# parsakzr/medvae-disentangled-multimodal

Measured on AMD Instinct MI355X. Metric: training images/sec (whole node) + ELBO parity, multimodal CVAE 64×64 bs=256, higher is better.
Workload: dtype fp32 (3xBF16 MFMA, fp32 accumulate); 1 GPU; ConditionalVAE 64x64x3 train step (fwd+loss+bwd+clip+adamw); model=ConditionalVAE, params=927333315, global_batch=256, per_gpu_batch=256, resolution=64, parallelism=dp1, rccl_world_size=1, step_launch=eager

## Files before the change

include/medvae_hip.h:

```cpp
#ifndef MEDVAE_HIP_H
#define MEDVAE_HIP_H

#include <stddef.h>

#ifdef __cplusplus
extern "C" {
#endif

#define MVAE_OK 0
#define MVAE_EINVAL (-1)
#define MVAE_EWORKSPACE (-2)

const char* mvae_last_error(void);
int mvae_abi_version(void);

int mvae_set_math_mode(int mode);
int mvae_get_math_mode(void);
int mvae_set_dropout_salt(const void* salt_dev);

#define MVAE_CONV_WSPLIT 16
#define MVAE_CONV_XSPLIT 32
#define MVAE_CONV_DYSPLIT 64
#define MVAE_CONV_BF16 128
#define MVAE_CONV_PLANAR 256
// ... 40 lines not shown
int mvae_conv2d_wgrad_upsample_nhwc(const float* dy, const float* x, float* dw, float* dbias, float beta, int nb,
                                    int h, int w_, int cin, int cout, float* workspace, size_t workspace_bytes,
                                    void* stream);
size_t mvae_conv2d_wgrad_upsample_workspace_bytes(int nb, int h, int w_, int cin, int cout);

int mvae_winograd_weight_transform(const float* w, void* u, int cin, int cout, int dgrad, int tile, void* stream);
int mvae_winograd_input_transform(const float* x, void* v, int nb, int h, int w, int c, int x_split, int tile,
                                  void* stream);
int mvae_winograd_input_transform_gn(const float* x, const float* scale, const float* shift, int silu, void* v, int nb,
                                     int h, int w, int c, int tile, void* stream);
int mvae_winograd_gemm(const void* v, const void* u, float* m, long long tiles, int k_in, int n_out, int tile,
                       void* stream);
int mvae_winograd_output_transform(const float* m, const float* bias, const float* residual, float* y, double* gn_part,
                                   int nb, int h, int w, int n, int tile, void* stream);
int mvae_winograd_output_gnbwd(const float* m, float* dx, const float* x, const float* mean, const float* rstd,
                               const float* gamma, const float* beta, int groups, int silu, double* part, int nb, int h,
                               int w, int n, int tile, void* stream);
int mvae_winograd_dy_transform(const float* dy, void* d, int nb, int h, int w, int k, int dy_split, int tile,
                               void* stream);
int mvae_winograd_dy_transforms(const float* dy, void* v, void* d, int nb, int h, int w, int k, int dy_split, int tile,
                                void* stream);
int mvae_winograd_wgrad_gemm(const void* d, const void* v, float* m, long long tiles, int cout, int cin, int tile,
                             float* workspace, size_t workspace_bytes, void* stream);
int mvae_winograd_wgrad_output(const float* m, float* dw, float beta, int cout, int cin, int tile, void* stream);
int mvae_winograd_upsample_weights(const float* w, float* kc, int cin, int cout, void* stream);
int mvae_winograd_upsample_fold(const float* dkc, float* dw, float beta, int cin, int cout, void* stream);
int mvae_winograd_output_transform_upsample(const float* m, const float* bias, float* y, int nb, int h, int w, int cout,
                                            int tile, void* stream);
int mvae_winograd_dy_transforms_upsample(const float* dy, void* v, void* d, int nb, int h, int w, int cout, int tile,
                                         void* stream);

int mvae_split_bf16(const float* x, void* y, long long n, void* stream);
int mvae_pack_bf16(const float* x, void* y, long long n, void* stream);
int mvae_pack_bf16_colsum(const float* x, void* y, long long rows, int n, float* out, float beta, void* workspace,
                          size_t workspace_bytes, void* stream);
int mvae_split_planar(const float* x, void* y, long long n, void* stream);
int mvae_split_planar_colsum(const float* x, void* y, long long rows, int n, float* out, float beta, void* workspace,
                             size_t workspace_bytes, void* stream);

int mvae_conv_weight_transpose(const float* w, float* wt, int cout, int kh, int kw, int cin, int split, void* stream);
typedef struct {
  const float* w;
  float* wt;
  int cout, rs, cin, split;
  int block0, pad0;
} mvae_wt_desc;
int mvae_conv_weight_transpose_batched(const mvae_wt_desc* table, int n, int total_blocks, void* stream);
// ... 183 lines not shown
```

medvae_disentangled_multimodal_amd/_lib.py:

```python
from __future__ import annotations

import ctypes
import os
from ctypes import c_double, c_float, c_int, c_longlong, c_size_t, c_uint64, c_void_p

_HERE = os.path.dirname(os.path.abspath(__file__))
LIB_PATH = os.environ.get("MVAE_HIP_LIB", os.path.join(_HERE, "libmvae_hip.so"))

P = c_void_p
I = c_int
L = c_longlong
F = c_float
D = c_double
Z = c_size_t

SIGNATURES = {
    "mvae_last_error": (ctypes.c_char_p, []),
    "mvae_abi_version": (I, []),
    "mvae_set_math_mode": (I, [I]),
    "mvae_get_math_mode": (I, []),
    "mvae_set_dropout_salt": (I, [P]),
    "mvae_conv2d_nhwc": (I, [P, P, P, P, P, I, I, I, I, I, I, I, I, I, I, I, I, I, P]),
    "mvae_conv2d_direct32_nhwc": (I, [P, P, P, P, P, I, I, I, I, P]),
    "mvae_conv2d_ws_nhwc": (I, [P, P, P, P, P, I, I, I, I, I, I, I, I, I, I, I, I, I, P, Z, P]),
    "mvae_conv2d_split_workspace_bytes": (Z, [I, I, I, I, I, I, I]),
    "mvae_conv2d_gnstats_nhwc": (I, [P, P, P, P, P, I, I, I, I, I, I, I, I, I, I, I, I, I, P, P]),
    "mvae_conv2d_dgrad_gnbwd_nhwc": (I, [P, P, P, I, I, I, I, I, I, I, I, I, I, I, I, P, P, P, P, P, I, I, P, P]),
    "mvae_conv2d_wgrad_nhwc": (I, [P, P, P, P, F, I, I, I, I, I, I, I, I, I, I, I, I, I, P, Z, P]),
    "mvae_winograd_weight_transform": (I, [P, P, I, I, I, I, P]),
    "mvae_winograd_input_transform": (I, [P, P, I, I, I, I, I, I, P]),
    "mvae_winograd_input_transform_gn": (I, [P, P, P, I, P, I, I, I, I, I, P]),
    "mvae_group_norm_stats_nhwc": (I, [P, P, P, P, P, P, P, P, I, I, I, I, F, P, Z, P]),
    "mvae_group_norm_apply_nhwc": (I, [P, P, P, P, I, I, I, I, I, P]),
    "mvae_winograd_gemm": (I, [P, P, P, L, I, I, I, P]),
    "mvae_winograd_output_transform": (I, [P, P, P, P, P, I, I, I, I, I, P]),
    "mvae_winograd_output_gnbwd": (I, [P, P, P, P, P, P, P, I, I, P, I, I, I, I, I, P]),
    "mvae_winograd_dy_transform": (I, [P, P, I, I, I, I, I, I, P]),
    "mvae_winograd_dy_transforms": (I, [P, P, P, I, I, I, I, I, I, P]),
    "mvae_winograd_wgrad_gemm": (I, [P, P, P, L, I, I, I, P, Z, P]),
    "mvae_winograd_wgrad_output": (I, [P, P, F, I, I, I, P]),
    "mvae_winograd_upsample_weights": (I, [P, P, I, I, P]),
    "mvae_winograd_upsample_fold": (I, [P, P, F, I, I, P]),
    "mvae_winograd_output_transform_upsample": (I, [P, P, P, I, I, I, I, I, P]),
    "mvae_winograd_dy_transforms_upsample": (I, [P, P, P, I, I, I, I, I, P]),
    "mvae_conv2d_wgrad_workspace_bytes": (Z, [I, I, I, I, I, I, I]),
    "mvae_conv2d_wgrad_small_cout_nhwc": (I, [P, P, P, P, F, I, I, I, I, I, I, P, Z, P]),
    "mvae_conv2d_wgrad_small_cout_workspace_bytes": (Z, [I, I]),
    "mvae_conv2d_wgrad_direct_nhwc": (I, [P, P, P, P, F, I, I, I, I, I, I, P, Z, P]),
    "mvae_conv2d_wgrad_direct_workspace_bytes": (Z, [I, I, I, I, I]),
    "mvae_conv_weight_transpose": (I, [P, P, I, I, I, I, I, P]),
    "mvae_conv_weight_transpose_batched": (I, [P, I, I, P]),
    "mvae_conv_weight_upsample_dgrad": (I, [P, P, I, I, I, P]),
    "mvae_conv2d_dgrad_stride2_nhwc": (I, [P, P, P, I, I, I, I, I, I, I, I, I, I, I, I, P, Z, P]),
    "mvae_split_bf16": (I, [P, P, L, P]),
    "mvae_pack_bf16": (I, [P, P, L, P]),
    "mvae_pack_bf16_colsum": (I, [P, P, L, I, P, F, P, Z, P]),
    "mvae_split_planar": (I, [P, P, L, P]),
    "mvae_split_planar_colsum": (I, [P, P, L, I, P, F, P, Z, P]),
    "mvae_conv2d_upsample_nhwc": (I, [P, P, P, P, P, I, I, I, I, I, I, P]),
    "mvae_conv_weight_upsample_fwd": (I, [P, P, I, I, I, P]),
    "mvae_conv2d_wgrad_upsample_nhwc": (I, [P, P, P, P, F, I, I, I, I, I, P, Z, P]),
    "mvae_conv2d_wgrad_upsample_workspace_bytes": (Z, [I, I, I, I, I]),
    "mvae_bias_grad": (I, [P, L, I, L, P, F, P, Z, P]),
# ... 141 lines not shown
```

medvae_disentangled_multimodal_amd/csrc/gemm_core.h:

```cpp
#pragma once
#include "common.h"
#include <algorithm>
#include <stdlib.h>
#include <type_traits>

namespace mvae {

enum { A_ROWK = 0, A_COLM = 1, A_CONV_FWD = 2, A_CONV_UPS = 3, A_CONV_DGRAD = 4, A_CONV_SUBPIX = 5, A_COLM_PIX = 6,
       A_CONV_FWD_SPLIT = 7, A_CONV_DGRAD_SPLIT = 8, A_COLM_SPLIT = 9, A_ROWK_SPLIT = 10 };
enum { B_ROWK = 0, B_COLN = 1, B_WGRAD_FWD = 2, B_WGRAD_UPS = 3, B_WGRAD_SUBPIX = 4, B_ROWK_SPLIT = 5,
       B_WGRAD_FWD_SPLIT = 6, B_WGRAD_P2 = 7, B_WGRAD_P2_SPLIT = 8, B_COLN_SPLIT = 9 };
enum { MODE_FWD = 0, MODE_UPS = 1, MODE_DGRAD = 2, MODE_SUBPIX = 3 };

constexpr int BK = 32;
template <int MF> using acc_of = typename std::conditional<MF == 32, f32x16, f32x4>::type;
template <int MF> constexpr int ks_of() { return BK / (MF == 32 ? 16 : 32); }
template <int MF> constexpr int nr_of() { return MF == 32 ? 16 : 4; }
__device__ __forceinline__ int row_swz(int r) { return ((r >> 2) ^ (r >> 3) ^ (r >> 4)) & 1; }
__device__ __forceinline__ int col_swz(int kr) { return ((kr >> 3) & 1) << 4; }
__device__ __forceinline__ int row_off(int r, int kc) { return r * 40 + (((kc >> 1) ^ row_swz(r)) << 3) + ((kc & 1) << 2); }
constexpr int MVAE_CONV_WSPLIT = 16;
constexpr int MVAE_CONV_XSPLIT = 32;
constexpr int MVAE_CONV_DYSPLIT = 64;
constexpr int MVAE_CONV_BF16 = 128;
constexpr int MVAE_CONV_PLANAR = 256;
constexpr int MVAE_CONV_DGRAD_DIRECT = 512;

struct Magic {
  unsigned m;
  int sh;
};
inline Magic make_magic(int d) {
  int l = 0;
  while ((1LL << l) < d) ++l;
  return Magic{(unsigned)(((1ULL << (31 + l)) / (unsigned long long)d) + 1ULL), 31 + l};
}
__device__ __forceinline__ int mdiv(int n, Magic mg) {
  return (int)(((unsigned long long)(unsigned)n * mg.m) >> mg.sh);
}

struct GemmArgs {
  int M, N, K;
  int batch, splits, k_split;
  const float* A; long long lda, sA;
  const float* B; long long ldb, sB;
  float* C; long long ldc, sC;
// ... 1587 lines not shown
    }
  }
}

template <int BM, int BN, int WGM, int WGN, int AK, int VA, int BKIND, int VB, int PREC>
__global__ void __launch_bounds__(64 * WGM * WGN) gemm3x_persist_kernel(GemmArgs a) {
  constexpr int NT = 64 * WGM * WGN;
  constexpr int MF = (MVAE_COL_MF16 && mf_of(AK) == 32) ? 16 : mf_of(AK);
  static_assert(MF == 16 && (PREC == 0 || PREC == 3), "persistent GEMM: 16x16x32 tiles, 3xBF16 or exact fp32");
  constexpr int KS = ks_of<MF>(), NR = nr_of<MF>();
  using acc_t = acc_of<MF>;
  using LA = Loader<AK, BM, VA, NT, true, PREC>;
  using LB = Loader<BKIND, BN, VB, NT, false, PREC>;
  using IA = Img<BM, LA::COL>;
  using IB = Img<BN, LB::COL>;
  constexpr int BUF = IA::SIZE + IB::SIZE;
  constexpr int TM = BM / WGM / MF, TN = BN / WGN / MF;
  static_assert(TM % 2 == 0, "persistent GEMM: the 16-B epilogue stages half of the wave's rows at a time");
  __shared__ __attribute__((aligned(16))) __bf16 lds[2 * BUF];

  const int tid = threadIdx.x, lane = tid & 63, wid = tid >> 6;
  const int wm = wid / WGN, wn = wid - wm * WGN;
  const int arow = wm * (BM / WGM), brow = wn * (BN / WGN);
  const int ntile = a.tiles_m * a.tiles_n, total = ntile * a.batch, grid = (int)gridDim.x;
  int lin = blockIdx.x;
  if (grid >= 16) {
    const int xcd = lin & 7, q = grid >> 3, r = grid & 7;
    lin = (xcd < r ? xcd * (q + 1) : r * (q + 1) + (xcd - r) * q) + (lin >> 3);
  }
  auto locate = [&](int l, int& m0, int& n0, int& bidx) {
    bidx = l / ntile;
    const int tile = l - bidx * ntile;
    int tm, tn;
    if (a.xcd_groups > 1 && a.tiles_n > 1) {
      const int gw = (a.tiles_n + a.xcd_groups - 1) / a.xcd_groups;
      const int ng = (a.tiles_n + gw - 1) / gw;
      const int g = min(tile / (a.tiles_m * gw), ng - 1);
      const int rem = tile - g * a.tiles_m * gw;
      const int width = g == ng - 1 ? a.tiles_n - g * gw : gw;
      tm = rem / width;
      tn = g * gw + (rem - tm * width);
    } else {
      tm = tile / a.tiles_n;
      tn = tile - tm * a.tiles_n;
    }
    m0 = tm * BM;
    n0 = tn * BN;
  };
  const int nt = (a.K + BK - 1) / BK;

  LA la;
  LB lb;
  auto prefetch = [&](int l) {
    int m0, n0, bidx;
    locate(l, m0, n0, bidx);
    la.init(a, a.A + bidx * a.sA, m0, 0, tid, bidx);
    lb.init(a, a.B + bidx * a.sB, n0, 0, tid, bidx);
    la.load(a);
    lb.load(a);
  };
  acc_t acc[TM][TN];
  auto compute = [&](const __bf16* Ai) {
    const __bf16* Bi = Ai + IA::SIZE;
#pragma unroll
    for (int ks = 0; ks < KS; ++ks) {
      bf16x8 bh[TN], bl[TN];
#pragma unroll
      for (int j = 0; j < TN; ++j) {
        bh[j] = read_frag<BN, LB::COL, MF>(Bi, brow + j * MF, ks, lane);
        bl[j] = read_frag<BN, LB::COL, MF>(Bi + IB::PLANE, brow + j * MF, ks, lane);
      }
#pragma unroll
      for (int i = 0; i < TM; ++i) {
        const bf16x8 ah = read_frag<BM, LA::COL, MF>(Ai, arow + i * MF, ks, lane);
        const bf16x8 al = read_frag<BM, LA::COL, MF>(Ai + IA::PLANE, arow + i * MF, ks, lane);
#pragma unroll
        for (int j = 0; j < TN; ++j) mma<PREC>(acc[i][j], ah, al, bh[j], bl[j]);
      }
    }
  };

  prefetch(lin);
  for (int l = lin;;) {
    int m0, n0, bidx;
    locate(l, m0, n0, bidx);
    const int lnext = l + grid;
    const bool more = lnext < total;
#pragma unroll
    for (int i = 0; i < TM; ++i)
#pragma unroll
      for (int j = 0; j < TN; ++j)
#pragma unroll
        for (int r = 0; r < NR; ++r) acc[i][j][r] = 0.f;
    la.store(lds);
    lb.store(lds + IA::SIZE);
    if (nt > 1) {
      la.advance();
      lb.advance();
      la.load(a);
      lb.load(a);
    }
    __syncthreads();
    int t = 0;
    constexpr int STEPS = KS * TM;
    constexpr int NSL = LA::NS + LB::NS;
#ifndef MVAE_NO_PRIO
    if (NT >= 512 && wid >= (NT / 64) / 2) __builtin_amdgcn_s_setprio(1);
#endif
// ... 41 lines not shown
            bh[j] = read_frag<BN, LB::COL, MF>(Bi, brow + j * MF, 1, lane);
            bl[j] = read_frag<BN, LB::COL, MF>(Bi + IB::PLANE, brow + j * MF, 1, lane);
          }
        }
        stage(st);
        __builtin_amdgcn_sched_barrier(0);
      }
      __syncthreads();
    }
#ifndef MVAE_NO_PRIO
    __builtin_amdgcn_s_setprio(0);
#endif
    if (t + 1 < nt) {
      __bf16* nb = lds + ((t & 1) ^ 1) * BUF;
      la.store(nb);
      lb.store(nb + IA::SIZE);
      compute(lds + (t & 1) * BUF);
      __syncthreads();
      ++t;
    }
    compute(lds + (t & 1) * BUF);
    if (more) prefetch(lnext);

    {
      constexpr int WR = BM / WGM, WC = BN / WGN, HR = WR / 2, PE = WC + 4;
      static_assert((NT / 64) * HR * PE * 4 <= 4 * BUF, "epilogue staging exceeds the LDS");
      constexpr int C4 = WC / 4, RPI = 64 / C4;
      float* stg = (float*)lds + wid * HR * PE;
      const __amdgpu_buffer_rsrc_t cr = make_rsrc(a.C + bidx * a.sC, a.c_bytes);
      const int c4 = lane % C4, rsub = lane / C4;
      const int col = n0 + brow + c4 * 4;
      __syncthreads();
#pragma unroll
      for (int pass = 0; pass < 2; ++pass) {
#pragma unroll
        for (int i = 0; i < TM / 2; ++i)
#pragma unroll
          for (int j = 0; j < TN; ++j)
#pragma unroll
            for (int r = 0; r < NR; ++r)
              stg[(i * 16 + acc_row<MF>(r, lane)) * PE + j * 16 + (lane & 15)] = acc[pass * (TM / 2) + i][j][r];
        __syncthreads();
#pragma unroll
        for (int k = 0; k < HR / RPI; ++k) {
          const int lr = k * RPI + rsub;
          const float4 s4 = *(const float4*)(stg + lr * PE + c4 * 4);
// ... 292 lines not shown
```

medvae_disentangled_multimodal_amd/csrc/winograd.hip:

```cpp
#include "gemm_core.h"

namespace mvae {

__device__ __forceinline__ float4 f4add(float4 a, float4 b) { return float4{a.x + b.x, a.y + b.y, a.z + b.z, a.w + b.w}; }

template <int MT>
__host__ __device__ constexpr float wino_bt(int i, int j) {
  if constexpr (MT == 2) {
    constexpr float m[4][4] = {{1, 0, -1, 0}, {0, 1, 1, 0}, {0, -1, 1, 0}, {0, 1, 0, -1}};
    return m[i][j];
  } else {
    constexpr float m[6][6] = {{4, 0, -5, 0, 1, 0},  {0, -4, -4, 1, 1, 0}, {0, 4, -4, -1, 1, 0},
                               {0, -2, -1, 2, 1, 0}, {0, 2, -1, -2, 1, 0}, {0, 4, 0, -5, 0, 1}};
    return m[i][j];
  }
}
template <int MT>
__host__ __device__ constexpr float wino_g(int i, int j) {
  if constexpr (MT == 2) {
    constexpr float m[4][3] = {{1, 0, 0}, {0.5f, 0.5f, 0.5f}, {0.5f, -0.5f, 0.5f}, {0, 0, 1}};
    return m[i][j];
  } else {
    constexpr float m[6][3] = {{0.25f, 0, 0},
                               {-1.f / 6, -1.f / 6, -1.f / 6},
// ... 577 lines not shown
#pragma unroll
  for (int i = 0; i < AL; ++i)
#pragma unroll
    for (int j = 0; j < AL; ++j) mv[i][j] = bload4(mr, (unsigned)(t * K4 + k4) * 16u + (unsigned)(i * AL + j) * mplane);
  constexpr auto at = [](int i, int k) { return wino_at<MT>(i, k); };
  float4 r[MT][AL];
#pragma unroll
  for (int j = 0; j < AL; ++j) wlin<MT, AL>(&r[0][j], AL, &mv[0][j], AL, at);
#pragma unroll
  for (int a = 0; a < MT; ++a) {
    float4 o[MT];
    wlin<MT, AL>(o, 1, &r[a][0], 1, at);
    const int row = ti * MT + a;
#pragma unroll
    for (int e = 0; e < MT; ++e) {
      const int col = tj * MT + e;
      const unsigned off =
          ((unsigned)((b * 2 * p.H + 2 * row + (pq >> 1)) * 2 * p.W + 2 * col + (pq & 1)) * (unsigned)N + c4 * 4) * 4u;
      bstore4(yr, (row < p.H && col < p.W) ? off : OOB, f4add(o[e], bv));
    }
  }
}

template <int MT>
__global__ void __launch_bounds__(256) wino_wout_kernel(const float* __restrict__ m, float* __restrict__ dw, float beta,
                                                        int cout, int cin) {
  constexpr int AL = MT + 2;
  const int C4 = cin >> 2;
  const long long idx = (long long)blockIdx.x * blockDim.x + threadIdx.x;
  if (idx >= (long long)cout * C4) return;
  const long long mn = (long long)cout * cin;
  float4 mv[AL][AL];
#pragma unroll
  for (int i = 0; i < AL; ++i)
#pragma unroll
    for (int j = 0; j < AL; ++j) mv[i][j] = *(const float4*)(m + (i * AL + j) * mn + idx * 4);
  constexpr auto gt = [](int r, int i) { return wino_g<MT>(i, r); };
  float4 r[3][AL], o[3][3];
#pragma unroll
  for (int j = 0; j < AL; ++j) wlin<3, AL>(&r[0][j], AL, &mv[0][j], AL, gt);
#pragma unroll
  for (int i = 0; i < 3; ++i) wlin<3, AL>(&o[i][0], 1, &r[i][0], 1, gt);
  const int k = (int)(idx / C4), c4 = (int)(idx - (long long)k * C4);
#pragma unroll
  for (int i = 0; i < 3; ++i)
#pragma unroll
    for (int j = 0; j < 3; ++j) {
      float4* q = (float4*)(dw + (((long long)k * 3 + i) * 3 + j) * cin + c4 * 4);
      float4 val = o[i][j];
      if (beta != 0.f) {
        const float4 old = *q;
        val = float4{fmaf(beta, old.x, val.x), fmaf(beta, old.y, val.y), fmaf(beta, old.z, val.z),
                     fmaf(beta, old.w, val.w)};
      }
      *q = val;
    }
}

static long long wino_tiles(int nb, int h, int w, int mt) {
  return (long long)nb * ((h + mt - 1) / mt) * ((w + mt - 1) / mt);
}

static bool wino_geom_ok(int mt, int nb, int h, int w, int cin, int cout) {
// ... 90 lines not shown
    if (tile == 2) hipLaunchKernelGGL(wino_out_any_kernel<2>, g, dim3(256), 0, st, p);
    else hipLaunchKernelGGL(wino_out_any_kernel<4>, g, dim3(256), 0, st, p);
    return launch_status();
  }
  const int wseg = std::min(p.W, 32);
  if (tile == 2) {
    if (wseg == 8) wino_out_go<2, 8>(p, gnb, st);
    else if (wseg == 16) wino_out_go<2, 16>(p, gnb, st);
    else wino_out_go<2, 32>(p, gnb, st);
  } else {
    if (wseg == 8) wino_out_go<4, 8>(p, gnb, st);
    else if (wseg == 16) wino_out_go<4, 16>(p, gnb, st);
    else wino_out_go<4, 32>(p, gnb, st);
  }
  return launch_status();
}

template <int CFG, int AK, int BKIND>
static bool persist_cfg(GemmArgs& a, hipStream_t st) {
  constexpr int BM = 256, BN = CFG == T256x256 ? 256 : 128;
  constexpr int WGM = CFG == T256x128 ? 4 : 2, WGN = CFG == T256x256 ? 4 : 2;
  a.tiles_m = cdiv(a.M, BM);
  a.tiles_n = cdiv(a.N, BN);
  const long long total = (long long)a.tiles_m * a.tiles_n * a.batch, slots = 256LL * resident_of(CFG);
  if (total <= slots || total > (1LL << 30)) return false;
  if (a.xcd_groups <= 0) a.xcd_groups = xcd_groups_env();
  const dim3 grid((unsigned)slots), block(64 * WGM * WGN);
  if (math_mode() == MATH_FP32) {
    if constexpr (CFG == T256x256) return false;
    else hipLaunchKernelGGL((gemm3x_persist_kernel<BM, BN, WGM, WGN, AK, 4, BKIND, 4, 0>), grid, block, 0, st, a);
  } else {
    hipLaunchKernelGGL((gemm3x_persist_kernel<BM, BN, WGM, WGN, AK, 4, BKIND, 4, 3>), grid, block, 0, st, a);
  }
  return true;
}
template <int AK, int BKIND>
static bool launch_persist(GemmArgs& a, hipStream_t st, int cfg) {
  static_assert(AK == A_ROWK_SPLIT && BKIND == B_ROWK_SPLIT, "persistent GEMM: pre-split ROW x ROW operands");
#ifdef MVAE_W4
  return false;
#else
  if (getenv("MVAE_NO_PERSISTENT_GEMM") != nullptr || math_mode() == MATH_BF16 || a.splits != 1 || a.bias || a.res ||
      a.beta != 0.f || a.out_remap || a.gn_part || a.gnb_part || a.bias_ws || (a.N & 3) || (a.ldc & 3) || (a.sC & 3) ||
      !al16(a.C) || vec_epi_disabled())
    return false;
  if (cfg == T256x256) return persist_cfg<T256x256, AK, BKIND>(a, st);
  if (cfg == T256x128) return persist_cfg<T256x128, AK, BKIND>(a, st);
  return false;
#endif
}

}

using namespace mvae;

extern "C" {

int mvae_winograd_weight_transform(const float* w, void* u, int cin, int cout, int dgrad, int tile, void* stream) {
  if (!w || !u || cin <= 0 || cout <= 0 || cin % 4 || cout % 4 || !al16(w) || !al16(u) || (tile != 2 && tile != 4)) {
    set_error("winograd_weight_transform: cin, cout multiples of 4, 16-B aligned w / u, tile 2 or 4");
    return MVAE_EINVAL;
  }
  hipStream_t st = (hipStream_t)stream;
  const int sf = wino_sf();
  if (tile == 2) WINO_GO(wt_go, 2, w, u, cin, cout, dgrad, st);
  else WINO_GO(wt_go, 4, w, u, cin, cout, dgrad, st);
  return launch_status();
}

int mvae_winograd_input_transform(const float* x, void* v, int nb, int h, int w, int c, int x_split, int tile,
                                  void* stream) {
  if (!x || !v || !wino_geom_ok(tile, nb, h, w, c, c) || !al16(x) || !al16(v)) {
// ... 116 lines not shown
  hipStream_t st = (hipStream_t)stream;
  const int sf = wino_sf();
  if (tile == 2) WINO_GO(dy_go, 2, dy, nullptr, d, nb, h, w, k, dy_split, false, st);
  else WINO_GO(dy_go, 4, dy, nullptr, d, nb, h, w, k, dy_split, false, st);
  return launch_status();
}

int mvae_winograd_dy_transforms(const float* dy, void* v, void* d, int nb, int h, int w, int k, int dy_split, int tile,
                                void* stream) {
  if (!dy || !v || !d || !wino_geom_ok(tile, nb, h, w, k, k) || !al16(dy) || !al16(v) || !al16(d)) {
    set_error("winograd_dy_transforms: tile 2 or 4, k %% 4 == 0, 16-B aligned");
    return MVAE_EINVAL;
  }
  if (!wino_split_in_ok(dy_split)) return MVAE_EINVAL;
  hipStream_t st = (hipStream_t)stream;
  const int sf = wino_sf();
  if (tile == 2) WINO_GO(dy_go, 2, dy, v, d, nb, h, w, k, dy_split, true, st);
  else WINO_GO(dy_go, 4, dy, v, d, nb, h, w, k, dy_split, true, st);
  return launch_status();
}

int mvae_winograd_wgrad_gemm(const void* d, const void* v, float* m, long long tiles, int cout, int cin, int tile,
                             float* workspace, size_t workspace_bytes, void* stream) {
  if (!d || !v || !m || tiles <= 0 || cout <= 0 || cin <= 0 || cout % 4 || cin % 4 || !al16(d) || !al16(v) || !al16(m) ||
      tiles * std::max(cout, cin) * 4 > MAX_DESC_BYTES || tiles > (1LL << 30) || (tile != 2 && tile != 4)) {
    set_error("winograd_wgrad_gemm: cout, cin multiples of 4, 16-B aligned, one position < 4 GiB, tile 2 or 4");
    return MVAE_EINVAL;
  }
  const bool pk = wino_sf() == 2;
  if (pk && (cout % 8 || cin % 8)) {
    set_error("winograd_wgrad_gemm: the bf16 (packed) operands need cout, cin %% 8 == 0");
    return MVAE_EINVAL;
  }
  const unsigned eb = pk ? 2u : 4u;
  GemmArgs a{};
  a.M = cout; a.N = cin; a.K = (int)tiles; a.batch = (tile + 2) * (tile + 2);
  a.A = (const float*)d; a.lda = cout; a.sA = tiles * cout;
  a.B = (const float*)v; a.ldb = cin; a.sB = tiles * cin;
  a.C = m; a.ldc = cin; a.sC = (long long)cout * cin;
  a.alpha = 1.f; a.beta = 0.f;
  a.a_bytes = (unsigned)(tiles * cout * eb); a.b_bytes = (unsigned)(tiles * cin * eb);
  a.c_bytes = (unsigned)((long long)cout * cin * 4);
  const int cfg = choose_tile(a, true, workspace != nullptr);
  plan_splits(a, cfg, workspace, workspace_bytes);
  if (pk) wgrad_dma(B_COLN, a, (hipStream_t)stream, cfg, 4);
  else launch_big<A_COLM_SPLIT, 4, B_COLN_SPLIT, 4>(a, (hipStream_t)stream, cfg);
  return gemm_finish(a, (hipStream_t)stream);
}

int mvae_winograd_upsample_weights(const float* w, float* kc, int cin, int cout, void* stream) {
  if (!w || !kc || cin <= 0 || cout <= 0 || cin % 4 || !al16(w) || !al16(kc)) {
    set_error("winograd_upsample_weights: cin %% 4 == 0, 16-B aligned");
    return MVAE_EINVAL;
  }
  hipLaunchKernelGGL(wino_ups_weights_kernel, dim3(egrid256(4LL * cout * (cin / 4))), dim3(256), 0, (hipStream_t)stream,
                     w, kc, cout, cin);
  return launch_status();
}

int mvae_winograd_upsample_fold(const float* dkc, float* dw, float beta, int cin, int cout, void* stream) {
  if (!dkc || !dw || cin <= 0 || cout <= 0 || cin % 4 || !al16(dkc) || !al16(dw)) {
    set_error("winograd_upsample_fold: cin %% 4 == 0, 16-B aligned");
    return MVAE_EINVAL;
  }
  hipLaunchKernelGGL(wino_ups_fold_kernel, dim3(egrid256((long long)cout * (cin / 4))), dim3(256), 0,
                     (hipStream_t)stream, dkc, dw, beta, cout, cin);
  return launch_status();
}

int mvae_winograd_output_transform_upsample(const float* m, const float* bias, float* y, int nb, int h, int w, int cout,
// ... 6 lines not shown
  WinoOut p{};
  p.m = m; p.bias = bias; p.y = y;
  p.groups = 1; p.nb = nb; p.H = h; p.W = w; p.N = cout;
  const dim3 g(egrid256(wino_tiles(nb, h, w, tile) * cout));
  if (tile == 2) hipLaunchKernelGGL(wino_out_ups_kernel<2>, g, dim3(256), 0, (hipStream_t)stream, p);
  else hipLaunchKernelGGL(wino_out_ups_kernel<4>, g, dim3(256), 0, (hipStream_t)stream, p);
  return launch_status();
}

int mvae_winograd_dy_transforms_upsample(const float* dy, void* v, void* d, int nb, int h, int w, int cout, int tile,
                                         void* stream) {
  if (!dy || !d || cout % 4 || !wino_geom_ok(tile, nb, h, w, 4 * cout, 4 * cout) || !al16(dy) || !al16(d) ||
      (v && !al16(v))) {
    set_error("winograd_dy_transforms_upsample: tile 2 or 4, cout %% 4 == 0, 16-B aligned, operands < 4 GiB");
    return MVAE_EINVAL;
  }
  hipStream_t st = (hipStream_t)stream;
  const int sf = wino_sf(), k = 4 * cout;
  if (tile == 2) WINO_GO(dy_go, 2, dy, v, d, nb, h, w, k, 0, v != nullptr, st, true);
  else WINO_GO(dy_go, 4, dy, v, d, nb, h, w, k, 0, v != nullptr, st, true);
  return launch_status();
}

int mvae_winograd_wgrad_output(const float* m, float* dw, float beta, int cout, int cin, int tile, void* stream) {
  if (!m || !dw || cout <= 0 || cin <= 0 || cin % 4 || !al16(m) || !al16(dw) || (tile != 2 && tile != 4)) {
    set_error("winograd_wgrad_output: cin %% 4 == 0, 16-B aligned, tile 2 or 4");
    return MVAE_EINVAL;
  }
  const dim3 g(egrid256((long long)cout * (cin / 4)));
  if (tile == 2)
    hipLaunchKernelGGL(wino_wout_kernel<2>, g, dim3(256), 0, (hipStream_t)stream, m, dw, beta, cout, cin);
  else
    hipLaunchKernelGGL(wino_wout_kernel<4>, g, dim3(256), 0, (hipStream_t)stream, m, dw, beta, cout, cin);
  return launch_status();
}

}
```

medvae_disentangled_multimodal_amd/ops.py:

```python
from __future__ import annotations

import ctypes
import math
import os
import weakref
from dataclasses import dataclass
from typing import Optional, Tuple

import torch

from . import _lib

CL = torch.channels_last


def _stream(t: torch.Tensor) -> int:
    return torch.cuda.current_stream(t.device).cuda_stream


def _ptr(t: Optional[torch.Tensor]):
    return None if t is None else t.data_ptr()


def _check(t: torch.Tensor, name: str = "tensor"):
# ... 112 lines not shown
        return self.kh == 1 and self.kw == 1 and self.stride == 1 and not self.upsample and \
            self.pad_t == self.pad_l == self.pad_b == self.pad_r == 0


def _krsc(w: torch.Tensor) -> torch.Tensor:
    return w if w.is_contiguous(memory_format=CL) else w.contiguous(memory_format=CL)


def _subpixel_upsample(g: ConvGeom) -> bool:
    return g.upsample and g.kh == 3 and g.kw == 3 and g.stride == 1 and \
        g.pad_t == g.pad_l == g.pad_b == g.pad_r == 1 and SUBPIXEL_UPSAMPLE


SUBPIXEL_UPSAMPLE = os.environ.get("MVAE_NO_SUBPIXEL") is None
STRIDE2_CLASSES = os.environ.get("MVAE_NO_STRIDE2_CLASSES") is None
WEIGHT_SPLIT = os.environ.get("MVAE_NO_WEIGHT_SPLIT") is None
SMALL_COUT_WGRAD = os.environ.get("MVAE_NO_SMALL_COUT_WGRAD") is None
DIRECT_WGRAD = os.environ.get("MVAE_NO_DIRECT_WGRAD") is None
DIRECT_WGRAD_COUT = (32, 64) if os.environ.get("MVAE_DIRECT_WGRAD_C64") is not None else (32,)
MVAE_CONV_WSPLIT = 16
MVAE_CONV_XSPLIT = 32
MVAE_CONV_DYSPLIT = 64
MVAE_CONV_DGRAD_DIRECT = 512
DIRECT32 = os.environ.get("MVAE_NO_DIRECT32") is None


def _direct32(g, c: int, co: int, wd: int) -> bool:
    return (DIRECT32 and c == 32 and co == 32 and g.kh == 3 and g.kw == 3 and g.stride == 1 and not g.upsample and
            (g.pad_t, g.pad_l, g.pad_b, g.pad_r) == (1, 1, 1, 1) and wd <= 62)
DY_SPLIT = os.environ.get("MVAE_DY_SPLIT") is not None
DY_SPLIT_MIN = 1 << 18


def _al16(*ts) -> bool:
    return all(t.data_ptr() % 16 == 0 for t in ts)


WINOGRAD = os.environ.get("MVAE_NO_WINOGRAD") is None
WINOGRAD_MIN_C = int(os.environ.get("MVAE_WINOGRAD_MIN_C", "512"))
WINOGRAD_MIN_C_WIDE = int(os.environ.get("MVAE_WINOGRAD_MIN_C_WIDE", "256"))
WINOGRAD_TILE = int(os.environ.get("MVAE_WINOGRAD_TILE", "4"))
if WINOGRAD_TILE not in (2, 4):
    raise ValueError("MVAE_WINOGRAD_TILE must be 2 or 4")


WINOGRAD_EXACT = os.environ.get("MVAE_NO_WINOGRAD_EXACT") is None
# ... 751 lines not shown
        ws = ARENA.get("ws", nbytes, dy.device)
        _lib.call("mvae_conv2d_wgrad_direct_nhwc", dy.data_ptr(), x.data_ptr(), dw.data_ptr(), _ptr(db), float(beta),
                  n, h, wd, c, co, int(x_split), ws.data_ptr(), ws.numel(), st)
        return db is not None
    if not deferred and not x_split and _wino_ups_wgrad_ok(g, x, dy, dw):
        mt = _wtile()
        pos = (mt + 2) ** 2
        dev = dy.device
        kept = {e[4]: e[0] for e in wino_v or () if e[1] == mt and e[2] == x.data_ptr() and e[3] == x._version}
        kept_d = {e[4]: e[0] for e in wino_d or () if e[1] == mt and e[2] == dy.data_ptr() and e[3] == dy._version}
        dkc = ARENA.get("wups_dk", 4 * co * 9 * c * 4, dev)
        for i, (b0, b1) in enumerate(_wino_chunks(n, h, wd, max(c, 4 * co))):
            nb, t = b1 - b0, _wino_tiles(b1 - b0, h, wd)
            v, dt = kept.get((b0, b1)), kept_d.get((b0, b1))
            if dt is None:
                dt = ARENA.get("wino_d", _wel() * pos * t * 4 * co, dev)
                _lib.call("mvae_winograd_dy_transforms_upsample", dy[b0:b1].data_ptr(), None, dt.data_ptr(), nb, h, wd,
                          co, mt, st)
            if v is None:
                v = ARENA.get("wino_v", _wel() * pos * t * c, dev)
                _lib.call("mvae_winograd_input_transform", x[b0:b1].data_ptr(), v.data_ptr(), nb, h, wd, c, 0, mt, st)
            m = ARENA.get("wino_mw", 4 * pos * 4 * co * c, dev)
            ws = ARENA.get("ws", _lib.query("mvae_gemm_workspace_bytes", 4 * co, c, t, pos), dev)
            _lib.call("mvae_winograd_wgrad_gemm", dt.data_ptr(), v.data_ptr(), m.data_ptr(), t, 4 * co, c, mt,
                      ws.data_ptr(), ws.numel(), st)
            _lib.call("mvae_winograd_wgrad_output", m.data_ptr(), dkc.data_ptr(), 0.0 if i == 0 else 1.0, 4 * co, c, mt,
                      st)
        _lib.call("mvae_winograd_upsample_fold", dkc.data_ptr(), dw.data_ptr(), float(beta), c, co, st)
        return False
    if not deferred and _subpixel_upsample(g):
        nbytes = _lib.query("mvae_conv2d_wgrad_upsample_workspace_bytes", n, h, wd, c, co)
        ws = ARENA.get("ws", nbytes, dy.device)
        _lib.call("mvae_conv2d_wgrad_upsample_nhwc", dy.data_ptr(), x.data_ptr(), dw.data_ptr(), _ptr(db),
                  float(beta), n, h, wd, c, co, ws.data_ptr(), ws.numel(), st)
        return db is not None
    if _wino_wgrad_ok(g, x if lazy is None else lazy.x, dy, dw, dys):
        mt = _wtile()
        pos = (mt + 2) ** 2
        dev = dy.device
        dya = dys if dys is not None else dy
        kept = {}
        for e in wino_v or ():
            if e[1] == mt and e[2] == x.data_ptr() and e[3] == x._version:
                kept[e[4]] = e[0]
        kept_d = {}
        for e in wino_d or ():
            if e[1] == mt and e[2] == dya.data_ptr() and e[3] == dya._version:
                kept_d[e[4]] = e[0]
        for i, (b0, b1) in enumerate(_wino_chunks(n, h, wd, max(c, co))):
            nb, t = b1 - b0, _wino_tiles(b1 - b0, h, wd)
            v = kept.get((b0, b1))
            dt = kept_d.get((b0, b1))
            m = ARENA.get("wino_mw", 4 * pos * co * c, dev)
            ws = ARENA.get("ws", _lib.query("mvae_gemm_workspace_bytes", co, c, t, pos), dev)
            if dt is None:
                dt = ARENA.get("wino_d", _wel() * pos * t * co, dev)
                _lib.call("mvae_winograd_dy_transform", dya[b0:b1].data_ptr(), dt.data_ptr(), nb, h, wd, co,
                          int(dys is not None), mt, st)
            if v is None and lazy is not None:
                v = ARENA.get("wino_v", _wel() * pos * t * c, dev)
                _lib.call("mvae_winograd_input_transform_gn", lazy.x[b0:b1].data_ptr(), lazy.scale[b0 * c:].data_ptr(),
                          lazy.shift[b0 * c:].data_ptr(), lazy.silu, v.data_ptr(), nb, h, wd, c, mt, st)
            elif v is None:
                v = ARENA.get("wino_v", _wel() * pos * t * c, dev)
                _lib.call("mvae_winograd_input_transform", x[b0:b1].data_ptr(), v.data_ptr(), nb, h, wd, c,
                          int(x_split), mt, st)
            _lib.call("mvae_winograd_wgrad_gemm", dt.data_ptr(), v.data_ptr(), m.data_ptr(), t, co, c, mt,
                      ws.data_ptr(), ws.numel(), st)
            _lib.call("mvae_winograd_wgrad_output", m.data_ptr(), dw.data_ptr(), float(beta) if i == 0 else 1.0, co, c,
                      mt, st)
        return False
    nbytes = _lib.query("mvae_conv2d_wgrad_workspace_bytes", n, c, co, g.kh, g.kw, ho, wo)
    ws = ARENA.get("ws", nbytes, dy.device)
    mode = (1 if g.upsample else 0) | (MVAE_CONV_XSPLIT if x_split else 0)
    dya = dy
    if dys is not None and co % 4 == 0:
        mode |= MVAE_CONV_DYSPLIT
        dya = dys
        db = None
    _lib.call("mvae_conv2d_wgrad_nhwc", dya.data_ptr(), x.data_ptr(), dw.data_ptr(), _ptr(db), float(beta), n, h, wd,
              c, co, g.kh, g.kw, g.stride, g.pad_t, g.pad_l, ho, wo, mode, ws.data_ptr(), ws.numel(), st)
    return db is not None


def bias_grad_raw(dy2d_ptr, rows, n, out, beta, device, stream):
    nbytes = _lib.query("mvae_bias_grad_workspace_bytes", rows, n)
    ws = ARENA.get("bias", nbytes, device)
    _lib.call("mvae_bias_grad", dy2d_ptr, rows, n, n, out.data_ptr(), float(beta), ws.data_ptr(), ws.numel(), stream)


class DxSum:
    __slots__ = ("n", "left", "buf")

# ... 1383 lines not shown
```

Measured before the change: 788.0 images/s.

## Fuse Winograd wgrad split-K reduction into output transform; add persistent split-K GEMM

The Winograd weight-gradient GEMM now leaves its split-K partials in the workspace instead of reducing them in a separate finish pass. The output-transform kernel sums the partials itself before applying the inverse transform. A persistent-kernel path for the column-major split-K GEMM is also added, which writes partials straight from the accumulators. This removes one reduction kernel and one round trip of the M buffer per chunk. In exchange the output kernel reads splits times more data, and the persistent kernel gains split-K bookkeeping.

Result: no change. 791.9 images/s, median of 4 (+0.5%).

```diff
diff --git a/include/medvae_hip.h b/include/medvae_hip.h
--- a/include/medvae_hip.h
+++ b/include/medvae_hip.h
@@ -86,7 +86,11 @@
                                 void* stream);
 int mvae_winograd_wgrad_gemm(const void* d, const void* v, float* m, long long tiles, int cout, int cin, int tile,
                              float* workspace, size_t workspace_bytes, void* stream);
-int mvae_winograd_wgrad_output(const float* m, float* dw, float beta, int cout, int cin, int tile, void* stream);
+#define MVAE_WINO_KEEP_PARTIALS 256
+int mvae_winograd_wgrad_splits(long long tiles, int cout, int cin, int tile, const float* workspace,
+                               size_t workspace_bytes);
+int mvae_winograd_wgrad_output(const float* m, const float* partials, int splits, float* dw, float beta, int cout,
+                               int cin, int tile, void* stream);
 int mvae_winograd_upsample_weights(const float* w, float* kc, int cin, int cout, void* stream);
 int mvae_winograd_upsample_fold(const float* dkc, float* dw, float beta, int cin, int cout, void* stream);
 int mvae_winograd_output_transform_upsample(const float* m, const float* bias, float* y, int nb, int h, int w, int cout,
diff --git a/medvae_disentangled_multimodal_amd/_lib.py b/medvae_disentangled_multimodal_amd/_lib.py
--- a/medvae_disentangled_multimodal_amd/_lib.py
+++ b/medvae_disentangled_multimodal_amd/_lib.py
@@ -38,7 +38,8 @@
     "mvae_winograd_dy_transform": (I, [P, P, I, I, I, I, I, I, P]),
     "mvae_winograd_dy_transforms": (I, [P, P, P, I, I, I, I, I, I, P]),
     "mvae_winograd_wgrad_gemm": (I, [P, P, P, L, I, I, I, P, Z, P]),
-    "mvae_winograd_wgrad_output": (I, [P, P, F, I, I, I, P]),
+    "mvae_winograd_wgrad_splits": (I, [L, I, I, I, P, Z]),
+    "mvae_winograd_wgrad_output": (I, [P, P, I, P, F, I, I, I, P]),
     "mvae_winograd_upsample_weights": (I, [P, P, I, I, P]),
     "mvae_winograd_upsample_fold": (I, [P, P, F, I, I, P]),
     "mvae_winograd_output_transform_upsample": (I, [P, P, P, I, I, I, I, I, P]),
diff --git a/medvae_disentangled_multimodal_amd/csrc/gemm_core.h b/medvae_disentangled_multimodal_amd/csrc/gemm_core.h
--- a/medvae_disentangled_multimodal_amd/csrc/gemm_core.h
+++ b/medvae_disentangled_multimodal_amd/csrc/gemm_core.h
@@ -22,6 +22,7 @@
 constexpr int MVAE_CONV_WSPLIT = 16;
 constexpr int MVAE_CONV_XSPLIT = 32;
 constexpr int MVAE_CONV_DYSPLIT = 64;
+constexpr int MVAE_WINO_KEEP_PARTIALS = 256;
 constexpr int MVAE_CONV_BF16 = 128;
 constexpr int MVAE_CONV_PLANAR = 256;
 constexpr int MVAE_CONV_DGRAD_DIRECT = 512;
@@ -1655,15 +1656,20 @@
   const int tid = threadIdx.x, lane = tid & 63, wid = tid >> 6;
   const int wm = wid / WGN, wn = wid - wm * WGN;
   const int arow = wm * (BM / WGM), brow = wn * (BN / WGN);
-  const int ntile = a.tiles_m * a.tiles_n, total = ntile * a.batch, grid = (int)gridDim.x;
+  constexpr bool SPLITK = LA::COL;
+  static_assert(LA::COL == LB::COL, "persistent GEMM: ROW x ROW or COL x COL images");
+  const int nsplit = SPLITK ? a.splits : 1;
+  const int ntile = a.tiles_m * a.tiles_n, total = ntile * a.batch * nsplit, grid = (int)gridDim.x;
   int lin = blockIdx.x;
   if (grid >= 16) {
     const int xcd = lin & 7, q = grid >> 3, r = grid & 7;
     lin = (xcd < r ? xcd * (q + 1) : r * (q + 1) + (xcd - r) * q) + (lin >> 3);
   }
-  auto locate = [&](int l, int& m0, int& n0, int& bidx) {
-    bidx = l / ntile;
-    const int tile = l - bidx * ntile;
+  auto locate = [&](int l, int& m0, int& n0, int& bidx, int& split) {
+    const int z = l / ntile;
+    const int tile = l - z * ntile;
+    bidx = SPLITK ? z / nsplit : z;
+    split = SPLITK ? z - bidx * nsplit : 0;
     int tm, tn;
     if (a.xcd_groups > 1 && a.tiles_n > 1) {
       const int gw = (a.tiles_n + a.xcd_groups - 1) / a.xcd_groups;
@@ -1680,15 +1686,19 @@
     m0 = tm * BM;
     n0 = tn * BN;
   };
-  const int nt = (a.K + BK - 1) / BK;
+  auto ktiles = [&](int split) {
+    const int kb = split * a.k_split;
+    return SPLITK ? (min(a.K, kb + a.k_split) - kb + BK - 1) / BK : (a.K + BK - 1) / BK;
+  };
 
   LA la;
   LB lb;
   auto prefetch = [&](int l) {
-    int m0, n0, bidx;
-    locate(l, m0, n0, bidx);
-    la.init(a, a.A + bidx * a.sA, m0, 0, tid, bidx);
-    lb.init(a, a.B + bidx * a.sB, n0, 0, tid, bidx);
+    int m0, n0, bidx, split;
+    locate(l, m0, n0, bidx, split);
+    const int kb = SPLITK ? split * a.k_split : 0;
+    la.init(a, a.A + bidx * a.sA, m0, kb, tid, bidx);
+    lb.init(a, a.B + bidx * a.sB, n0, kb, tid, bidx);
     la.load(a);
     lb.load(a);
   };
@@ -1715,8 +1725,9 @@
 
   prefetch(lin);
   for (int l = lin;;) {
-    int m0, n0, bidx;
-    locate(l, m0, n0, bidx);
+    int m0, n0, bidx, split;
+    locate(l, m0, n0, bidx, split);
+    const int nt = ktiles(split);
     const int lnext = l + grid;
     const bool more = lnext < total;
 #pragma unroll
@@ -1804,6 +1815,26 @@
     compute(lds + (t & 1) * BUF);
     if (more) prefetch(lnext);
 
+    if (SPLITK && nsplit > 1) {
+      const __amdgpu_buffer_rsrc_t ws =
+          make_rsrc(a.ws + ((long long)bidx * nsplit + split) * a.M * a.N, (unsigned)(a.M * a.N * 4u));
+#pragma unroll
+      for (int j = 0; j < TN; ++j) {
+        const int col = n0 + brow + j * MF + (lane & (MF - 1));
+#pragma unroll
+        for (int i = 0; i < TM; ++i)
+#pragma unroll
+          for (int r = 0; r < NR; ++r) {
+            const int row = m0 + arow + i * MF + acc_row<MF>(r, lane);
+            const bool ok = row < a.M && col < a.N;
+            bstore1(ws, ok ? ((unsigned)row * a.N + col) * 4u : OOB, acc[i][j][r]);
+          }
+      }
+      __syncthreads();
+      if (!more) break;
+      l = lnext;
+      continue;
+    }
     {
       constexpr int WR = BM / WGM, WC = BN / WGN, HR = WR / 2, PE = WC + 4;
       static_assert((NT / 64) * HR * PE * 4 <= 4 * BUF, "epilogue staging exceeds the LDS");
diff --git a/medvae_disentangled_multimodal_amd/csrc/winograd.hip b/medvae_disentangled_multimodal_amd/csrc/winograd.hip
--- a/medvae_disentangled_multimodal_amd/csrc/winograd.hip
+++ b/medvae_disentangled_multimodal_amd/csrc/winograd.hip
@@ -623,23 +623,49 @@
   }
 }
 
-template <int MT>
-__global__ void __launch_bounds__(256) wino_wout_kernel(const float* __restrict__ m, float* __restrict__ dw, float beta,
-                                                        int cout, int cin) {
-  constexpr int AL = MT + 2;
+template <int MT, bool SPLIT>
+__global__ void __launch_bounds__(256, SPLIT ? 2 : 1) wino_wout_kernel(const float* __restrict__ m, float* __restrict__ dw, float beta,
+                                                        int cout, int cin, int splits) {
+  constexpr int AL = MT + 2, WZ = 4;
   const int C4 = cin >> 2;
   const long long idx = (long long)blockIdx.x * blockDim.x + threadIdx.x;
   if (idx >= (long long)cout * C4) return;
   const long long mn = (long long)cout * cin;
-  float4 mv[AL][AL];
-#pragma unroll
-  for (int i = 0; i < AL; ++i)
-#pragma unroll
-    for (int j = 0; j < AL; ++j) mv[i][j] = *(const float4*)(m + (i * AL + j) * mn + idx * 4);
   constexpr auto gt = [](int r, int i) { return wino_g<MT>(i, r); };
   float4 r[3][AL], o[3][3];
-#pragma unroll
-  for (int j = 0; j < AL; ++j) wlin<3, AL>(&r[0][j], AL, &mv[0][j], AL, gt);
+  if constexpr (SPLIT) {
+    const unsigned toff = (unsigned)idx * 16u;
+#pragma unroll
+    for (int j = 0; j < AL; ++j) {
+      float4 mc[AL];
+#pragma unroll
+      for (int i = 0; i < AL; ++i) mc[i] = float4{0.f, 0.f, 0.f, 0.f};
+      for (int z0 = 0; z0 < splits; z0 += WZ) {
+        float4 wv[AL][WZ];
+#pragma unroll
+        for (int i = 0; i < AL; ++i)
+#pragma unroll
+          for (int q = 0; q < WZ; ++q)
+            wv[i][q] = *(const float4*)((const char*)(m + ((long long)(i * AL + j) * splits + min(z0 + q, splits - 1)) * mn) + toff);
+#pragma unroll
+        for (int i = 0; i < AL; ++i)
+#pragma unroll
+          for (int q = 0; q < WZ; ++q) {
+            const float4 t = z0 + q < splits ? wv[i][q] : float4{0.f, 0.f, 0.f, 0.f};
+            mc[i].x += t.x; mc[i].y += t.y; mc[i].z += t.z; mc[i].w += t.w;
+          }
+      }
+      wlin<3, AL>(&r[0][j], AL, mc, 1, gt);
+    }
+  } else {
+    float4 mv[AL][AL];
+#pragma unroll
+    for (int i = 0; i < AL; ++i)
+#pragma unroll
+      for (int j = 0; j < AL; ++j) mv[i][j] = *(const float4*)(m + (i * AL + j) * mn + idx * 4);
+#pragma unroll
+    for (int j = 0; j < AL; ++j) wlin<3, AL>(&r[0][j], AL, &mv[0][j], AL, gt);
+  }
 #pragma unroll
   for (int i = 0; i < 3; ++i) wlin<3, AL>(&o[i][0], 1, &r[i][0], 1, gt);
   const int k = (int)(idx / C4), c4 = (int)(idx - (long long)k * C4);
@@ -776,17 +802,30 @@
   constexpr int WGM = CFG == T256x128 ? 4 : 2, WGN = CFG == T256x256 ? 4 : 2;
   a.tiles_m = cdiv(a.M, BM);
   a.tiles_n = cdiv(a.N, BN);
-  const long long total = (long long)a.tiles_m * a.tiles_n * a.batch, slots = 256LL * resident_of(CFG);
+  const long long total = (long long)a.tiles_m * a.tiles_n * a.batch * a.splits, slots = 256LL * resident_of(CFG);
   if (total <= slots || total > (1LL << 30)) return false;
   if (a.xcd_groups <= 0) a.xcd_groups = xcd_groups_env();
   const dim3 grid((unsigned)slots), block(64 * WGM * WGN);
   if (math_mode() == MATH_FP32) {
-    if constexpr (CFG == T256x256) return false;
+    if constexpr (CFG == T256x256 || AK == A_COLM_SPLIT) return false;
     else hipLaunchKernelGGL((gemm3x_persist_kernel<BM, BN, WGM, WGN, AK, 4, BKIND, 4, 0>), grid, block, 0, st, a);
   } else {
     hipLaunchKernelGGL((gemm3x_persist_kernel<BM, BN, WGM, WGN, AK, 4, BKIND, 4, 3>), grid, block, 0, st, a);
   }
   return true;
+}
+static bool launch_persist_wgrad(GemmArgs& a, hipStream_t st, int cfg) {
+#ifdef MVAE_W4
+  return false;
+#else
+  if (getenv("MVAE_NO_PERSISTENT_GEMM") != nullptr || math_mode() != MATH_3XBF16 || cfg != T256x256 || a.bias || a.res ||
+      a.beta != 0.f || a.out_remap || a.gn_part || a.gnb_part || a.bias_ws)
+    return false;
+  if (a.splits > 1 ? a.ws == nullptr
+                   : ((a.N & 3) || (a.ldc & 3) || (a.sC & 3) || !al16(a.C) || vec_epi_disabled()))
+    return false;
+  return persist_cfg<T256x256, A_COLM_SPLIT, B_COLN_SPLIT>(a, st);
+#endif
 }
 template <int AK, int BKIND>
 static bool launch_persist(GemmArgs& a, hipStream_t st, int cfg) {
@@ -802,6 +841,14 @@
   if (cfg == T256x128) return persist_cfg<T256x128, AK, BKIND>(a, st);
   return false;
 #endif
+}
+
+static int wgrad_plan(GemmArgs& a, long long tiles, int cout, int cin, int tile, const float* workspace,
+                      size_t workspace_bytes) {
+  a.M = cout; a.N = cin; a.K = (int)tiles; a.batch = (tile + 2) * (tile + 2);
+  const int cfg = choose_tile(a, true, workspace != nullptr);
+  plan_splits(a, cfg, const_cast<float*>(workspace), workspace_bytes);
+  return cfg;
 }
 
 }
@@ -964,6 +1011,8 @@
 
 int mvae_winograd_wgrad_gemm(const void* d, const void* v, float* m, long long tiles, int cout, int cin, int tile,
                              float* workspace, size_t workspace_bytes, void* stream) {
+  const bool keep = (tile & MVAE_WINO_KEEP_PARTIALS) != 0;
+  tile &= ~MVAE_WINO_KEEP_PARTIALS;
   if (!d || !v || !m || tiles <= 0 || cout <= 0 || cin <= 0 || cout % 4 || cin % 4 || !al16(d) || !al16(v) || !al16(m) ||
       tiles * std::max(cout, cin) * 4 > MAX_DESC_BYTES || tiles > (1LL << 30) || (tile != 2 && tile != 4)) {
     set_error("winograd_wgrad_gemm: cout, cin multiples of 4, 16-B aligned, one position < 4 GiB, tile 2 or 4");
@@ -976,18 +1025,31 @@
   }
   const unsigned eb = pk ? 2u : 4u;
   GemmArgs a{};
-  a.M = cout; a.N = cin; a.K = (int)tiles; a.batch = (tile + 2) * (tile + 2);
+  const int cfg = wgrad_plan(a, tiles, cout, cin, tile, workspace, workspace_bytes);
+  if (keep && a.splits > 1 && !al16(workspace)) {
+    set_error("winograd_wgrad_gemm: kept partials need a 16-B aligned workspace");
+    return MVAE_EINVAL;
+  }
   a.A = (const float*)d; a.lda = cout; a.sA = tiles * cout;
   a.B = (const float*)v; a.ldb = cin; a.sB = tiles * cin;
   a.C = m; a.ldc = cin; a.sC = (long long)cout * cin;
   a.alpha = 1.f; a.beta = 0.f;
   a.a_bytes = (unsigned)(tiles * cout * eb); a.b_bytes = (unsigned)(tiles * cin * eb);
   a.c_bytes = (unsigned)((long long)cout * cin * 4);
-  const int cfg = choose_tile(a, true, workspace != nullptr);
-  plan_splits(a, cfg, workspace, workspace_bytes);
   if (pk) wgrad_dma(B_COLN, a, (hipStream_t)stream, cfg, 4);
-  else launch_big<A_COLM_SPLIT, 4, B_COLN_SPLIT, 4>(a, (hipStream_t)stream, cfg);
+  else if (!launch_persist_wgrad(a, (hipStream_t)stream, cfg))
+    launch_big<A_COLM_SPLIT, 4, B_COLN_SPLIT, 4>(a, (hipStream_t)stream, cfg);
+  if (keep && a.splits > 1) return launch_status();
   return gemm_finish(a, (hipStream_t)stream);
+}
+
+int mvae_winograd_wgrad_splits(long long tiles, int cout, int cin, int tile, const float* workspace,
+                               size_t workspace_bytes) {
+  tile &= ~MVAE_WINO_KEEP_PARTIALS;
+  if (tiles <= 0 || tiles > (1LL << 30) || cout <= 0 || cin <= 0 || (tile != 2 && tile != 4)) return 1;
+  GemmArgs a{};
+  wgrad_plan(a, tiles, cout, cin, tile, workspace, workspace_bytes);
+  return a.splits;
 }
 
 int mvae_winograd_upsample_weights(const float* w, float* kc, int cin, int cout, void* stream) {
@@ -1040,16 +1102,22 @@
   return launch_status();
 }
 
-int mvae_winograd_wgrad_output(const float* m, float* dw, float beta, int cout, int cin, int tile, void* stream) {
-  if (!m || !dw || cout <= 0 || cin <= 0 || cin % 4 || !al16(m) || !al16(dw) || (tile != 2 && tile != 4)) {
-    set_error("winograd_wgrad_output: cin %% 4 == 0, 16-B aligned, tile 2 or 4");
+int mvae_winograd_wgrad_output(const float* m, const float* partials, int splits, float* dw, float beta, int cout,
+                               int cin, int tile, void* stream) {
+  const float* src = splits > 1 ? partials : m;
+  if (!src || !dw || cout <= 0 || cin <= 0 || cin % 4 || !al16(src) || !al16(dw) || (tile != 2 && tile != 4)) {
+    set_error("winograd_wgrad_output: cin %% 4 == 0, 16-B aligned m (partials when splits > 1), tile 2 or 4");
     return MVAE_EINVAL;
   }
   const dim3 g(egrid256((long long)cout * (cin / 4)));
-  if (tile == 2)
-    hipLaunchKernelGGL(wino_wout_kernel<2>, g, dim3(256), 0, (hipStream_t)stream, m, dw, beta, cout, cin);
-  else
-    hipLaunchKernelGGL(wino_wout_kernel<4>, g, dim3(256), 0, (hipStream_t)stream, m, dw, beta, cout, cin);
+  hipStream_t st = (hipStream_t)stream;
+  if (splits > 1) {
+    if (tile == 2) hipLaunchKernelGGL((wino_wout_kernel<2, true>), g, dim3(256), 0, st, src, dw, beta, cout, cin, splits);
+    else hipLaunchKernelGGL((wino_wout_kernel<4, true>), g, dim3(256), 0, st, src, dw, beta, cout, cin, splits);
+  } else {
+    if (tile == 2) hipLaunchKernelGGL((wino_wout_kernel<2, false>), g, dim3(256), 0, st, src, dw, beta, cout, cin, 1);
+    else hipLaunchKernelGGL((wino_wout_kernel<4, false>), g, dim3(256), 0, st, src, dw, beta, cout, cin, 1);
+  }
   return launch_status();
 }
 
diff --git a/medvae_disentangled_multimodal_amd/ops.py b/medvae_disentangled_multimodal_amd/ops.py
--- a/medvae_disentangled_multimodal_amd/ops.py
+++ b/medvae_disentangled_multimodal_amd/ops.py
@@ -158,6 +158,7 @@
 MVAE_CONV_XSPLIT = 32
 MVAE_CONV_DYSPLIT = 64
 MVAE_CONV_DGRAD_DIRECT = 512
+MVAE_WINO_KEEP_PARTIALS = 256
 DIRECT32 = os.environ.get("MVAE_NO_DIRECT32") is None
 
 
@@ -955,10 +956,11 @@
                 _lib.call("mvae_winograd_input_transform", x[b0:b1].data_ptr(), v.data_ptr(), nb, h, wd, c, 0, mt, st)
             m = ARENA.get("wino_mw", 4 * pos * 4 * co * c, dev)
             ws = ARENA.get("ws", _lib.query("mvae_gemm_workspace_bytes", 4 * co, c, t, pos), dev)
-            _lib.call("mvae_winograd_wgrad_gemm", dt.data_ptr(), v.data_ptr(), m.data_ptr(), t, 4 * co, c, mt,
-                      ws.data_ptr(), ws.numel(), st)
-            _lib.call("mvae_winograd_wgrad_output", m.data_ptr(), dkc.data_ptr(), 0.0 if i == 0 else 1.0, 4 * co, c, mt,
-                      st)
+            ns = _lib.query("mvae_winograd_wgrad_splits", t, 4 * co, c, mt, ws.data_ptr(), ws.numel())
+            _lib.call("mvae_winograd_wgrad_gemm", dt.data_ptr(), v.data_ptr(), m.data_ptr(), t, 4 * co, c,
+                      mt | MVAE_WINO_KEEP_PARTIALS, ws.data_ptr(), ws.numel(), st)
+            _lib.call("mvae_winograd_wgrad_output", m.data_ptr(), ws.data_ptr(), ns, dkc.data_ptr(),
+                      0.0 if i == 0 else 1.0, 4 * co, c, mt, st)
         _lib.call("mvae_winograd_upsample_fold", dkc.data_ptr(), dw.data_ptr(), float(beta), c, co, st)
         return False
     if not deferred and _subpixel_upsample(g):
@@ -998,10 +1000,11 @@
                 v = ARENA.get("wino_v", _wel() * pos * t * c, dev)
                 _lib.call("mvae_winograd_input_transform", x[b0:b1].data_ptr(), v.data_ptr(), nb, h, wd, c,
                           int(x_split), mt, st)
-            _lib.call("mvae_winograd_wgrad_gemm", dt.data_ptr(), v.data_ptr(), m.data_ptr(), t, co, c, mt,
-                      ws.data_ptr(), ws.numel(), st)
-            _lib.call("mvae_winograd_wgrad_output", m.data_ptr(), dw.data_ptr(), float(beta) if i == 0 else 1.0, co, c,
-                      mt, st)
+            ns = _lib.query("mvae_winograd_wgrad_splits", t, co, c, mt, ws.data_ptr(), ws.numel())
+            _lib.call("mvae_winograd_wgrad_gemm", dt.data_ptr(), v.data_ptr(), m.data_ptr(), t, co, c,
+                      mt | MVAE_WINO_KEEP_PARTIALS, ws.data_ptr(), ws.numel(), st)
+            _lib.call("mvae_winograd_wgrad_output", m.data_ptr(), ws.data_ptr(), ns, dw.data_ptr(),
+                      float(beta) if i == 0 else 1.0, co, c, mt, st)
         return False
     nbytes = _lib.query("mvae_conv2d_wgrad_workspace_bytes", n, c, co, g.kh, g.kw, ho, wo)
     ws = ARENA.get("ws", nbytes, dy.device)
```
